# cvlab-stonybrook/s-volsdf

Measured on AMD Instinct MI355X. Metric: rendered rays/sec (1024-ray batch, 128 samples), higher is better.
Workload: dtype f32 (every product, forward and backward, as three fp16 MFMA products of two-piece fp16 operands with f32 accumulate; activation blocks hold both pieces: float32 accuracy class); 1 GPU; configs[1]: VolOpt.train_step (forward + MVS prior lookup + loss + backward + clip/guard/Adam), train mode, fast=1: 1024 rays/GPU x 128 coarse + 98 composited samples + 2048 eikonal points, 8x256 SDF MLP + 4x256 radiance MLP; mode=train, mlp_precision=fp16x2, launch=eager launches, rays_per_gpu=1024, rays_total=1024

## Files before the change

### include/svolsdf_hip.h

```cpp
#ifndef SVOLSDF_HIP_H
#define SVOLSDF_HIP_H

#include <stddef.h>
#include <stdint.h>

#ifdef __cplusplus
extern "C" {
#endif

int svs_version(void);
const char* svs_last_error_string(void);

int svs_set_deterministic(int on);
int svs_get_deterministic(void);

int svs_rays_from_uv(const float* uv, const float* pose, const float* intrinsics, int n_rays, float* ray_dirs,
                     float* cam_loc, float* depth_scale, void* hip_stream);

int svs_eikonal_points(const float* uniform_points, const float* cam_loc, const float* z_eik, const float* ray_dirs,
                       int n_rays, float* points, void* hip_stream);
int svs_stage_in(const void* pinned_host, void* device, size_t bytes, void* hip_stream);
int svs_split_last(const float* z, int n_rays, int n, float* head, float* last, void* hip_stream);

enum { SVS_MMA_F32 = 0, SVS_MMA_F16X2 = 1, SVS_MMA_F16X2_HALF = 2 };
// ... 53 lines not shown
                   float* zbuf, float* feat_bar, float* absmax, void* hip_stream);
int svs_bg_sdf_bwd(int n_points, const float* d_out0, const float* feat_bar, const float* hbuf, const float* ghat7,
                   const float* stream, int precision, float* abuf, float* sbar_out, float* absmax, void* hip_stream);
int svs_composite_bg(int n_rays, int n_samples, int n_bg, const float* z, const float* z_max, const float* sdf,
                     const float* rgb, const float* normals, const float* depth_scale, const float* beta_param,
                     float beta_min, const float* z_bg, const float* bg_out0, const float* bg_rgb, const float* bg_depth,
                     float* weights, float* bg_trans, float* bg_weights, float* rgb_values, float* depth_values,
                     float* depth_values_all, float* depth_vals, float* normal_map, void* hip_stream);
int svs_composite_bg_bwd(int n_rays, int n_samples, int n_bg, const float* z, const float* z_max, const float* sdf,
                         const float* rgb, const float* depth_scale, const float* beta_param, float beta_min,
                         const float* z_bg, const float* bg_out0, const float* bg_rgb, const float* d_rgb_values,
                         const float* d_weights, const float* d_depth_values, const float* d_depth_all,
                         const float* bg_depth, float* d_sdf, float* d_rgb,
                         float* d_bg_out0, float* d_bg_rgb, float* d_beta_ray, float* d_beta_param, void* hip_stream);

typedef struct svs_wgrad_job {
  const float *a0, *b0; long long sa0, sb0;
  const float *a1, *b1; long long sa1, sb1;
  const float* b_extra; long long s_extra;
  int n_points, ldw;
  float *dW, *db;
  const float* absmax;
  const float *rec0, *rec1;
} svs_wgrad_job;
int svs_wgrad_multi(const svs_wgrad_job* jobs, int n_jobs, int precision, void* hip_stream);
int svs_wgrad(const float* a0, const float* b0, long long sa0, long long sb0, const float* a1, const float* b1,
              long long sa1, long long sb1, const float* b_extra, long long s_extra, int n_points, int precision,
              const float* absmax, const float* rec0, const float* rec1, float* dW, int ldw, float* db, void* hip_stream);

size_t svs_block_bytes(int n_points, int blocks_per_tile);
size_t svs_rgb_zbuf_bytes(int n_points);
size_t svs_sdf_ubuf_bytes(int n_points);
size_t svs_sdf_gbuf_bytes(int n_points);
int svs_rgb_bwd(int n_points, const float* d_rgb, const float* rgb, const float* rbuf, const float* stream, int precision,
                float* zbuf, float* feat_bar, float* d_normals, float* absmax, void* hip_stream);
int svs_sdf_bwd_a(const float* points, int n_points, const float* cam, int cam_stride, const float* dirs, const float* z,
                  int S, int n_rays, const float* d_grad, const unsigned char* clamp_mask, const float* hbuf,
                  const float* gbuf, const float* stream, int precision, float* ubuf, float* a2buf, float* pebuf,
                  float* absmax, void* hip_stream);
int svs_sdf_bwd_b(int n_points, const float* d_sdf, const unsigned char* clamp_mask, const float* feat_bar,
                  int n_feat_points, const float* hbuf, const float* gbuf, const float* a2buf, const float* ubuf,
                  const float* stream, int precision, float* abuf, float* sbar_out, float* absmax, void* hip_stream);
int svs_lin8_row0_grad(const float* hbuf, const float* ubuf, const float* sbar, int n_points, int precision, float* out257,
                       void* hip_stream);
int svs_unpack_wgrad(const float* dWk, const float* dbk, int ldw, int map, int rows, int cols, int row_off,
                     const float* weight_v, const float* weight_g, const float* row0, float* grad_v, float* grad_g,
                     float* grad_b, void* hip_stream);
// ... 205 lines not shown
```

### s-volsdf_amd/csrc/svs_wgrad.hip

```cpp
#include "svs_common.h"
#include "svs_mlp_layout.h"
#include "svs_ticket.h"
#include <cstdlib>

namespace svs {
namespace wgrad {

struct Pair {
  const float* a;
  const float* b;
  size_t stride_a, stride_b;
};

struct Args {
  Pair p[2];
  int n_pairs;
  int n_tiles;
  int n_valid_points;
  const float* b_extra;
  size_t stride_extra;
  float* dW;
  int ldw;
  float* db;
  det::Ticket ticket;
// ... 137 lines not shown
  __builtin_amdgcn_sched_barrier(0);
}
__device__ __forceinline__ unsigned lds_addr(const void* p) {
  return (unsigned)(unsigned long long)SVS_LDS(const void, p);
}

__device__ __forceinline__ void scale_from_absmax(const float* absmax, float& s, float& inv_s) {
  s = 1.0f; inv_s = 1.0f;
  if (!absmax) return;
  int e = (int)((__float_as_uint(*absmax) >> 23) & 0xff);
  e = e < 16 ? 16 : (e > 250 ? 250 : e);
  s = __uint_as_float((unsigned)(268 - e) << 23);
  inv_s = __uint_as_float((unsigned)(e - 14) << 23);
}

struct Job {
  Pair p[2];
  const float* rec[2];
  int n_pairs;
  int n_tiles;
  int n_valid_points;
  int b_tiles;
  int col0;
  float* dW;
  int ldw;
  float* db;
  const float* absmax;
  int wg_begin, wg_count;
  det::Ticket ticket;
};
constexpr int kMaxJobs = 20;
struct MultiArgs { Job job[kMaxJobs]; int n_jobs; int touch; int reverse; };
static_assert(sizeof(MultiArgs) <= 4096, "kernel arguments");

constexpr int kThreadsW = 512;

typedef const __attribute__((address_space(1))) void* gvoid;

template <bool GP>
__global__ __launch_bounds__(kThreadsW, 1) void wgrad_h2_multi_kernel(MultiArgs ma) {
  typedef Ring<GP> R;
  constexpr int kSlot = R::kSlot, kSlotAll = R::kSlotAll, kRing = R::kRing, kAhead = R::kAhead, kB = R::kB;
  extern __shared__ __attribute__((aligned(16))) unsigned char smem_h2[];
  int jj = 0;
  for (int q = 1; q < ma.n_jobs; ++q) if ((int)blockIdx.x >= ma.job[q].wg_begin) jj = q;
  const Job& a = ma.job[jj];
  const int wg = (int)blockIdx.x - a.wg_begin, nwg = a.wg_count;
  const int tid = threadIdx.x, lane = tid & 63;
  const int wave = __builtin_amdgcn_readfirstlane(tid >> 6);
  const bool narrow = a.b_tiles == 1;
  float s_grad, inv_s;
  scale_from_absmax(a.absmax, s_grad, inv_s);

  f32x16 acc[8];
#pragma unroll
  for (int i = 0; i < 8; ++i) acc[i] = (f32x16)(0.0f);
  float bsum = 0.0f;

  unsigned char* ring = smem_h2;

  const int rq = (lane & 15) >> 2, rp = lane & 3, rg = (lane >> 4) & 1, rh = lane >> 5;
  const int rd0 = 1024 * rg + 256 * rh + 128 * rg + 64 * (rp & 1) + 16 * rq + 8 * (rp >> 1);
  const int a_rd = 2048 * wave + rd0;
  const int rx0 = 64 * (8 * rh + rq) + 32 * rg + 8 * rp, rx1 = rx0 + 64 * 4;
  const int wp = lane & 31, whf = lane >> 5;
  const int wxoff = 64 * wp + 16 * (wave & 3) + 8 * whf;

  const bool two_pairs = a.n_pairs == 2;
  const int my_tiles = a.n_tiles > wg ? (a.n_tiles - 1 - wg) / nwg + 1 : 0;
  const int n_items = two_pairs ? 2 * my_tiles : my_tiles;
  const int n_valid = a.n_valid_points;
  const bool has_db = a.db != nullptr;
  const bool rev = ma.reverse != 0;
  const float* const pa0 = a.p[0].a; const float* const pb0 = a.p[0].b;
  const float* const pa1 = a.p[1].a; const float* const pb1 = a.p[1].b;
  const size_t sa0 = a.p[0].stride_a, sb0 = a.p[0].stride_b, sa1 = a.p[1].stride_a, sb1 = a.p[1].stride_b;
  const float* const rec0 = a.rec[0]; const float* const rec1 = a.rec[1];
  const bool has_scale = a.absmax != nullptr;
  auto tile_of = [&](int item) {
    const int k = two_pairs ? item >> 1 : item;
    return rev ? wg + (my_tiles - 1 - k) * nwg : wg + k * nwg;
  };

  auto issue = [&](int item) {
    const int t = tile_of(item), pi = two_pairs ? item & 1 : 0;
    const float* pa = (pi ? pa1 : pa0) + (size_t)t * (pi ? sa1 : sa0);
    const float* pb = (pi ? pb1 : pb0) + (size_t)t * (pi ? sb1 : sb0);
    unsigned char* slot = ring + (item % kRing) * kSlotAll;
#pragma unroll
    for (int j = 0; j < 2 * R::kPlanes; ++j) {
      const int piece = wave + 8 * j;
      __builtin_amdgcn_global_load_lds((gvoid)(reinterpret_cast<const f32x4*>(pa) + piece * 64 + lane),
                                       SVS_LDS(void, slot + piece * 1024), 16, 0, 0);
      if (!narrow)
        __builtin_amdgcn_global_load_lds((gvoid)(reinterpret_cast<const f32x4*>(pb) + piece * 64 + lane),
                                         SVS_LDS(void, slot + kB + piece * 1024), 16, 0, 0);
    }
    if (narrow)
      __builtin_amdgcn_global_load_lds((gvoid)(reinterpret_cast<const f32x4*>(pb) + (wave & 3) * 64 + lane),
                                       SVS_LDS(void, slot + kB + (wave & 3) * 1024), 16, 0, 0);
    if (has_scale)
      __builtin_amdgcn_global_load_lds((gvoid)((pi ? rec1 : rec0) + (size_t)t * 64 + lane),
                                       SVS_LDS(void, slot + kSlot + wave * 256), 4, 0, 0);
  };
  unsigned sink = 0;
  auto touch = [&](int item) {
    const int t = tile_of(item), pi = two_pairs ? item & 1 : 0;
    const Pair& p = a.p[pi];
    constexpr int kLines = R::kPlanes * (kPlane / 128);
    const int nb = narrow ? 32 : kLines;
    const float* q = tid < kLines ? p.a + (size_t)t * p.stride_a + tid * 32
                                  : p.b + (size_t)t * p.stride_b + (tid - kLines) * 32;
    if (tid < kLines + nb) asm volatile("global_load_dword %0, %1, off" : "+v"(sink) : "v"(q) : "memory");
  };
  const int ops = (narrow ? 2 * R::kPlanes + 1 : 4 * R::kPlanes) + (has_scale ? 1 : 0);

  auto stage_factors = [&](int item) {
    unsigned char* slot = ring + (item % kRing) * kSlotAll;
    const int t = tile_of(item);
    const int live = n_valid - t * 32;
    float f = 1.0f;
    if (has_scale) {
      float rec;
      lds_read32(rec, lds_addr(slot + kSlot + wave * 256 + 4 * wp));
      lds_wait();
      const unsigned eb = (__float_as_uint(rec) >> 23) & 0xff;
      if (eb >= 20 && eb <= 240) f = __builtin_fminf(s_grad * __uint_as_float((254u << 23) - __float_as_uint(rec)), 32768.0f);
    }
    if (wp >= live) f = 0.0f;
    if (lane < 32) asm volatile("ds_write_b16 %0, %1" :: "v"(lds_addr(slot + kSlot + kRecBytes + wave * 64 + 2 * lane)), "v"((_Float16)f) : "memory");
  };
  auto stage_narrow = [&](int item) {
    unsigned char* slot = ring + (item % kRing) * kSlotAll;
    if (tid < 256) {
      f32x4 v;
      lds_read128(v, lds_addr(slot + kB + tid * 16));
      lds_wait();
      f16x4 hi, mid;
#pragma unroll
      for (int j = 0; j < 4; ++j) {
        const _Float16 h = (_Float16)v[j];
        hi[j] = h;
        mid[j] = (_Float16)(v[j] - (float)h);
      }
      *SVS_LDS(f16x4, slot + kB + kNarrowImg + wxoff) = hi;
      *SVS_LDS(f16x4, slot + kB + kNarrowImg + kExtraPiece + wxoff) = mid;
    }
  };

  const f16x2 one2 = {(_Float16)1.0f, (_Float16)1.0f};

  for (int i0 = 0; i0 < kAhead && i0 < n_items; ++i0) issue(i0);
  const bool touching = GP && ma.touch;
  bool touched = false;
  if (touching && kAhead < n_items) { touch(kAhead); touched = true; }
  auto pre_stage = [&](int it) {
    const int left = n_items - 1 - it;
    const int later = (left < kAhead - 1 ? left : kAhead - 1) * ops;
    if (later == 10) asm volatile("s_waitcnt vmcnt(10)" ::: "memory");
    else if (later == 8) asm volatile("s_waitcnt vmcnt(8)" ::: "memory");
    else if (later == 6) asm volatile("s_waitcnt vmcnt(6)" ::: "memory");
    else if (later == 5) asm volatile("s_waitcnt vmcnt(5)" ::: "memory");
    else if (later == 4) asm volatile("s_waitcnt vmcnt(4)" ::: "memory");
    else if (later == 3) asm volatile("s_waitcnt vmcnt(3)" ::: "memory");
    else if (touched) asm volatile("s_waitcnt vmcnt(1)" ::: "memory");
    else asm volatile("s_waitcnt vmcnt(0)" ::: "memory");
    stage_factors(it);
  };
  for (int item = 0; item < n_items; ++item) {
    const int pi = two_pairs ? item & 1 : 0;
    const bool p0 = pi == 0;
    pre_stage(item);
    asm volatile("s_waitcnt lgkmcnt(0)\n\ts_barrier" ::: "memory");
    if (narrow) {
      stage_narrow(item);
      asm volatile("s_waitcnt lgkmcnt(0)\n\ts_barrier" ::: "memory");
    }
    auto issue_next = [&]() {
      if (item + kAhead < n_items) issue(item + kAhead);
      touched = false;
      if (touching && item + kAhead + 1 < n_items) { touch(item + kAhead + 1); touched = true; }
    };
    const unsigned la = lds_addr(ring + (item % kRing) * kSlotAll);
    const unsigned lb = la + kB;
    const unsigned ftab = la + kSlot + kRecBytes + wave * 64;
    const unsigned nimg = lb + kNarrowImg;
    const bool want_bias = has_db && p0;
    const bool two = narrow;
    Frag fa2[2], fam2[2];
    f32x4 fraw2[2];
#pragma unroll
    for (int ks = 0; ks < 2; ++ks) {
      tr_issue(fa2[ks], la + 512 * ks + a_rd, la + 512 * ks + (a_rd ^ 128));
      if (GP) tr_issue(fam2[ks], la + kPlane + 512 * ks + a_rd, la + kPlane + 512 * ks + (a_rd ^ 128));
      lds_read128(fraw2[ks], ftab + 32 * ks + 16 * rh);
    }
    issue_next();
    lds_wait();
#pragma unroll
    for (int ks = 0; ks < 2; ++ks) {
      const f16x8 ah = frag_of(fa2[ks]) * __builtin_bit_cast(f16x8, fraw2[ks]);
      const f16x8 am = GP ? frag_of(fam2[ks]) * __builtin_bit_cast(f16x8, fraw2[ks]) : ah;
      if (want_bias) {
#pragma unroll
        for (int j = 0; j < 4; ++j) {
          const f16x2 h2v = {ah[2 * j], ah[2 * j + 1]};
          bsum = __builtin_amdgcn_fdot2(h2v, one2, bsum, false);
          if (GP) {
            const f16x2 m2v = {am[2 * j], am[2 * j + 1]};
            bsum = __builtin_amdgcn_fdot2(m2v, one2, bsum, false);
          }
        }
      }
#pragma unroll
      for (int i = 0; i < 8; ++i) {
        if (i > 0 && narrow) break;
        Frag fh, fm;
        if (!narrow) {
          const unsigned rd = lb + 2048 * i + 512 * ks + rd0;
          tr_issue(fh, rd, rd ^ 128);
          if (GP) tr_issue(fm, rd + kPlane, (rd ^ 128) + kPlane);
        } else {
          tr_issue(fh, nimg + ks * 1024 + rx0, nimg + ks * 1024 + rx1);
          tr_issue(fm, nimg + kExtraPiece + ks * 1024 + rx0, nimg + kExtraPiece + ks * 1024 + rx1);
        }
        lds_wait();
        if (two || GP) acc[i] = __builtin_amdgcn_mfma_f32_32x32x16_f16(ah, frag_of(fm), acc[i], 0, 0, 0);
        if (GP) acc[i] = __builtin_amdgcn_mfma_f32_32x32x16_f16(am, frag_of(fh), acc[i], 0, 0, 0);
        acc[i] = __builtin_amdgcn_mfma_f32_32x32x16_f16(ah, frag_of(fh), acc[i], 0, 0, 0);
      }
    }
  }
  asm volatile("s_waitcnt vmcnt(0)" :: "v"(sink) : "memory");
  const int half = lane >> 5, col = lane & 31;
  det::wait_turn(a.ticket, wg);
#pragma unroll
  for (int i = 0; i < 8; ++i) {
    if (i > 0 && narrow) break;
#pragma unroll
    for (int r = 0; r < 16; ++r) {
      const int row = 32 * wave + rho(r) + 4 * half;
      const int c = a.col0 + 32 * i + col;
      if (c < a.ldw) atomicAdd(&a.dW[(size_t)row * a.ldw + c], acc[i][r] * inv_s);
    }
  }
  if (a.db) {
    bsum += __shfl_xor(bsum, 32);
    if (half == 0) atomicAdd(&a.db[32 * wave + col], bsum * inv_s);
  }
  det::pass_turn(a.ticket, wg);
}

}

}
}

using namespace svs;
using namespace svs::wgrad;
namespace h2 = svs::wgrad::h2;

extern "C" {

struct svs_wgrad_job {
  const float *a0, *b0; long long sa0, sb0;
  const float *a1, *b1; long long sa1, sb1;
  const float* b_extra; long long s_extra;
  int n_points, ldw;
  float *dW, *db;
  const float* absmax;
  const float *rec0, *rec1;
};

int svs_wgrad_multi(const svs_wgrad_job* jobs, int n_jobs, int precision, void* hip_stream) {
  if (!jobs || n_jobs < 1) { set_error("svs_wgrad_multi: no jobs"); return SVS_EINVAL; }
  int n_expanded = 0;
  for (int j = 0; j < n_jobs; ++j) n_expanded += jobs[j].b_extra ? 2 : 1;
  if (n_expanded > h2::kMaxJobs) { set_error("svs_wgrad_multi: at most %d jobs (b_extra counts twice)", h2::kMaxJobs); return SVS_EINVAL; }
  for (int j = 0; j < n_jobs; ++j) {
    const svs_wgrad_job& q = jobs[j];
    if (!q.a0 || !q.b0 || !q.dW || q.n_points <= 0 || q.ldw < 256 || q.ldw > 288 || (q.b_extra && q.ldw < 288) || (q.a1 && !q.b1)) {
      set_error("svs_wgrad_multi: bad argument in job %d", j); return SVS_EINVAL;
    }
    if (mlp::is_h2(precision) && q.absmax && (!q.rec0 || (q.a1 && !q.rec1))) {
      set_error("svs_wgrad_multi: job %d has absmax but no scale records", j); return SVS_EINVAL;
    }
  }
  hipStream_t s = (hipStream_t)hip_stream;
  if (mlp::is_h2(precision)) {
    const bool gp = precision == mlp::kFmtF16x2;
    h2::MultiArgs ma;
    int n = 0;
    long long work[h2::kMaxJobs], total = 0;
    for (int j = 0; j < n_jobs; ++j) {
      const svs_wgrad_job& q = jobs[j];
      h2::Job& J = ma.job[n];
      J.p[0] = Pair{q.a0, q.b0, (size_t)q.sa0, (size_t)q.sb0};
      J.rec[0] = q.rec0; J.rec[1] = q.rec1;
      J.n_pairs = 1;
      if (q.a1) { J.p[1] = Pair{q.a1, q.b1, (size_t)q.sa1, (size_t)q.sb1}; J.n_pairs = 2; }
      else { J.p[1] = J.p[0]; J.rec[1] = J.rec[0]; }
      J.n_tiles = (q.n_points + 31) / 32; J.n_valid_points = q.n_points;
      J.b_tiles = 8; J.col0 = 0; J.dW = q.dW; J.ldw = q.ldw; J.db = q.db; J.absmax = q.absmax;
      work[n] = (long long)J.n_tiles * J.n_pairs * 10;
      total += work[n++];
      if (q.b_extra) {
        h2::Job& X = ma.job[n];
        X = J;
        X.p[0].b = q.b_extra; X.p[0].stride_b = (size_t)q.s_extra; X.n_pairs = 1;
        X.b_tiles = 1; X.col0 = 256; X.db = nullptr;
        work[n] = (long long)X.n_tiles * 6;
        total += work[n++];
      }
    }
    ma.n_jobs = n;
    static const int touch_env = [] { const char* e = getenv("SVS_WGRAD_TOUCH"); return e ? atoi(e) : 0; }();
    ma.touch = touch_env;
    static const int reverse_env = [] { const char* e = getenv("SVS_WGRAD_REVERSE"); return e ? atoi(e) : 0; }();
    ma.reverse = reverse_env;
    (void)total;
    const int n_wg_total = 256;
    int count[h2::kMaxJobs];
    int used = 0;
    for (int j = 0; j < n; ++j) { count[j] = 1; ++used; }
    while (used < n_wg_total) {
      int best = -1;
      double load = 0.0;
      for (int j = 0; j < n; ++j) {
        if (count[j] >= ma.job[j].n_tiles) continue;
        const double l = (double)work[j] / count[j];
        if (l > load) { load = l; best = j; }
      }
      if (best < 0) break;
      ++count[best]; ++used;
// ... 72 lines not shown
```

### s-volsdf_amd/svs_hip/lib.py

```python
import ctypes
import os
from ctypes import POINTER, c_char_p, c_double, c_float, c_int, c_longlong, c_size_t, c_void_p

_HERE = os.path.dirname(os.path.abspath(__file__))
LIB_PATH = os.environ.get("SVS_LIB_PATH") or os.path.join(os.path.dirname(_HERE), "lib", "libsvolsdf_hip.so")

_lib = None


class SvsError(RuntimeError):
    pass


_P = c_void_p
_PP = POINTER(c_void_p)

class WGradJob(ctypes.Structure):
    _fields_ = [("a0", ctypes.c_void_p), ("b0", ctypes.c_void_p), ("sa0", ctypes.c_longlong), ("sb0", ctypes.c_longlong),
                ("a1", ctypes.c_void_p), ("b1", ctypes.c_void_p), ("sa1", ctypes.c_longlong), ("sb1", ctypes.c_longlong),
                ("b_extra", ctypes.c_void_p), ("s_extra", ctypes.c_longlong),
                ("n_points", ctypes.c_int), ("ldw", ctypes.c_int),
                ("dW", ctypes.c_void_p), ("db", ctypes.c_void_p), ("absmax", ctypes.c_void_p),
                ("rec0", ctypes.c_void_p), ("rec1", ctypes.c_void_p)]


class UnpackJob(ctypes.Structure):
    _fields_ = [("dWk", ctypes.c_void_p), ("dbk", ctypes.c_void_p), ("ldw", ctypes.c_int), ("map", ctypes.c_int),
                ("rows", ctypes.c_int), ("cols", ctypes.c_int), ("row_off", ctypes.c_int),
                ("weight_v", ctypes.c_void_p), ("weight_g", ctypes.c_void_p), ("row0", ctypes.c_void_p),
                ("grad_v", ctypes.c_void_p), ("grad_g", ctypes.c_void_p), ("grad_b", ctypes.c_void_p)]


SIGNATURES = {
    "svs_version": (c_int, []),
    "svs_set_deterministic": (c_int, [c_int]),
    "svs_get_deterministic": (c_int, []),
    "svs_last_error_string": (c_char_p, []),
    "svs_rays_from_uv": (c_int, [_P, _P, _P, c_int, _P, _P, _P, _P]),
    "svs_stream_bytes": (c_size_t, [c_int]),
    "svs_pack_stream": (c_int, [c_int, c_int, _PP, _PP, _PP, _P, _P, _P]),
    "svs_pack_workspace_bytes": (c_size_t, []),
    "svs_sdf_vals": (c_int, [_P, c_int, _P, c_int, _P, _P, c_int, c_int, _P, c_int, c_float, c_float, c_int, _P, _P,
                             c_int, c_int, _P]),
    "svs_sdf_hbuf_bytes": (c_size_t, [c_int]),
    "svs_sdf_gbuf_bytes": (c_size_t, [c_int]),
    "svs_feat_tiles_bytes": (c_size_t, [c_int]),
# ... 5 lines not shown
    "svs_block_bytes": (c_size_t, [c_int, c_int]),
    "svs_rgb_zbuf_bytes": (c_size_t, [c_int]),
    "svs_sdf_ubuf_bytes": (c_size_t, [c_int]),
    "svs_rgb_bwd": (c_int, [c_int, _P, _P, _P, _P, c_int, _P, _P, _P, _P, _P]),
    "svs_sdf_bwd_a": (c_int, [_P, c_int, _P, c_int, _P, _P, c_int, c_int, _P, _P, _P, _P, _P, c_int, _P, _P, _P,
                              _P, _P]),
    "svs_sdf_bwd_b": (c_int, [c_int, _P, _P, _P, c_int, _P, _P, _P, _P, _P, c_int, _P, _P, _P, _P]),
    "svs_lin8_row0_grad": (c_int, [_P, _P, _P, c_int, c_int, _P, _P]),
    "svs_unpack_wgrad": (c_int, [_P, _P, c_int, c_int, c_int, c_int, c_int, _P, _P, _P, _P, _P, _P, _P]),
    "svs_unpack_wgrad_multi": (c_int, [_P, c_int, _P]),
    "svs_sampler_ctl_bytes": (c_size_t, [c_int, c_int]),
    "svs_sampler_ctl_stride": (c_int, []),
    "svs_sampler_cap": (c_int, []),
    "svs_sampler_max_new": (c_int, []),
    "svs_sampler_init": (c_int, [_P, c_int, _P, c_int, c_int, c_float, c_float, c_int, c_float, _P, c_float, c_int,
                                 _P, _P, _P, _P, c_int, _P, _P]),
    "svs_sampler_round": (c_int, [c_int, c_int, c_int, c_int, c_int, c_int, c_int, _P, c_float, c_float, c_int, c_float,
                                  c_float, _P, _P, _P, _P, _P, _P, _P, c_int, _P, _P, _P, _P, _P, _P, _P, _P, _P, _P]),
    "svs_composite": (c_int, [c_int, c_int, _P, _P, _P, _P, _P, _P, c_float, _P, _P, _P, _P, _P, _P]),
    "svs_composite_bwd": (c_int, [c_int, c_int, _P, _P, _P, _P, _P, c_float, _P, _P, _P, _P, _P, _P, _P, _P]),
    "svs_wgrad": (c_int, [_P, _P, ctypes.c_longlong, ctypes.c_longlong, _P, _P, ctypes.c_longlong, ctypes.c_longlong,
                          _P, ctypes.c_longlong, c_int, c_int, _P, _P, _P, _P, c_int, _P, _P]),
    "svs_wgrad_multi": (c_int, [_P, c_int, c_int, _P]),
    "svs_bg_points": (c_int, [_P, c_int, _P, c_int, c_int, _P, c_float, _P, _P, _P, _P]),
    "svs_bg_sdf_eval": (c_int, [_P, c_int, _P, c_int, _P, _P, _P, _P, _P, _P]),
    "svs_bg_rgb_bwd": (c_int, [c_int, _P, _P, _P, _P, c_int, _P, _P, _P, _P]),
    "svs_bg_sdf_bwd": (c_int, [c_int, _P, _P, _P, _P, _P, c_int, _P, _P, _P, _P]),
    "svs_bg_rbuf_bytes": (c_size_t, [c_int]),
    "svs_bg_rgb_eval": (c_int, [c_int, _P, c_int, _P, _P, c_int, _P, _P, _P]),
    "svs_composite_bg_bwd": (c_int, [c_int, c_int, c_int, _P, _P, _P, _P, _P, _P, c_float, _P, _P, _P, _P, _P, _P, _P, _P,
                                     _P, _P, _P, _P, _P, _P, _P]),
    "svs_composite_bg": (c_int, [c_int, c_int, c_int, _P, _P, _P, _P, _P, _P, _P, c_float, _P, _P, _P, _P,
                                 _P, _P, _P, _P, _P, _P, _P, _P, _P]),
    "svs_adam_workspace_bytes": (c_size_t, []),
    "svs_clip_guard_adam": (c_int, [_P, _P, _P, _P, ctypes.c_longlong, c_int, _P, c_double, c_double, c_double, c_double,
                                    c_double, _P, _P, _P]),
    "svs_cost_lookup": (c_int, [_P, _P, _P, _P, c_int, c_int, c_int, c_int, c_int, c_float, c_float, POINTER(c_float),
                                _PP, _PP, _PP, POINTER(c_int), _P, _P, _P, _P, _P]),
    "svs_loss": (c_int, [c_int, c_int, c_int, _P, _P, _P, _P, _P, _P, _P, c_float, c_float, c_float, c_float, c_float,
                         c_float, c_int, c_float, c_int, c_int, _P, _P, _P, _P, _P, _P, _P, _P]),
    "svs_loss_workspace_bytes": (c_size_t, [c_int, c_int]),
    "svs_conv2d": (c_int, [_P, _P, _P, _P, c_int, _P, c_int, c_int, c_int, c_int, c_int, c_int, c_int, _P]),
    "svs_featurenet_fpn_workspace_bytes": (c_size_t, [c_int, c_int, c_int]),
    "svs_featurenet_fpn": (c_int, [_P, c_int, c_int, c_int, _P, _P, _P, _P, _P, _P, _P]),
    "svs_featurenet_fpn2": (c_int, [_P, c_int, c_int, c_int, _P, _P, _P, _P, _P, _P, _P, _P]),
    "svs_conv2d_mfma_supported": (c_int, [c_int, c_int, c_int, c_int]),
# ... 102 lines not shown
    "svs_lpips_workspace_bytes": (c_size_t, [c_int, c_int, c_int]),
    "svs_lpips_score": (c_int, [_P, _P, _P, c_int, c_int, c_int, _P, _P, _P, _P]),
})

ABI_VERSION = 101


def load():
    global _lib
    if _lib is not None:
        return _lib
    import torch
    if not os.path.exists(LIB_PATH):
        raise SvsError(f"{LIB_PATH} not found: run `python s-volsdf_amd/build.py` (there is no CPU fallback)")
    lib = ctypes.CDLL(LIB_PATH)
    for name, (res, args) in SIGNATURES.items():
        fn = getattr(lib, name)
        fn.restype = res
        fn.argtypes = args
    have = lib.svs_version()
    if have != ABI_VERSION:
        raise SvsError(f"{LIB_PATH} has ABI version {have}, this binding was written against {ABI_VERSION}: "
                       "rebuild with `python s-volsdf_amd/build.py --force`")
    if os.environ.get("SVS_DETERMINISTIC") == "1":
        lib.svs_set_deterministic(1)
    _lib = lib
    return lib


def deterministic():
    return bool(load().svs_get_deterministic())


def check(rc, what=""):
    if rc != 0:
        msg = load().svs_last_error_string()
        raise SvsError(f"{what} failed (code {rc}): {msg.decode() if msg else ''}")
```

### s-volsdf_amd/svs_hip/train.py

```python
import ctypes
import os

import torch

from . import lib as _lib
from .ops import _f32, _ptr, _ptr_array, _stream, default_precision, is_h2, F16X2, F16X2_HALF

KBLOCK = 128 * 64
KREC = 64


def block_stride(n_points):
    return ((n_points + 127) // 128) * 4 * KBLOCK
LDW = 288


def n_tiles_padded(n_points):
    return ((n_points + 127) // 128) * 4


def record_off(n_points, n_blocks, block):
    T = n_tiles_padded(n_points)
    return n_blocks * T * KBLOCK + block * T * KREC


def _off(t, n_floats):
    return t.data_ptr() + 4 * n_floats


class TrainStreams:
    def __init__(self, device, precision=None):
        L = _lib.load()
        self.precision = default_precision() if precision is None else int(precision)
        self.sdf = torch.empty(L.svs_stream_bytes(2) // 4, device=device)
        self.rgb = torch.empty(L.svs_stream_bytes(4) // 4, device=device)
        self.ws = torch.empty(L.svs_pack_workspace_bytes() // 4, device=device)

    def pack(self, sdf_params, rgb_params):
        L = _lib.load()
        sv, sg, sb = [[_f32(t) for t in x] if x is not None else None for x in sdf_params]
        rv, rg, rb = [[_f32(t) for t in x] if x is not None else None for x in rgb_params]
        self._keep = (sv, sg, sb, rv, rg, rb)
        st = _stream()
        _lib.check(L.svs_pack_stream(2, self.precision, _ptr_array(sv), _ptr_array(sg) if sg else None, _ptr_array(sb), _ptr(self.ws),
                                     _ptr(self.sdf), st), "svs_pack_stream(sdf train)")
        _lib.check(L.svs_pack_stream(4, self.precision, _ptr_array(rv), _ptr_array(rg) if rg else None, _ptr_array(rb), _ptr(self.ws),
                                     _ptr(self.rgb), st), "svs_pack_stream(rgb bwd)")


class WGradAccum:
    def __init__(self, device):
        n = [14 * 256 * LDW, 14 * 256, 260, 4]
        self.flat = torch.zeros(sum(n), device=device)
        parts = torch.split(self.flat, n)
        self.dWk = parts[0].view(14, 256, LDW)
        self.dbk = parts[1].view(14, 256)
        self.row0 = parts[2][:257]
        self.absmax = parts[3]

    def zero(self):
        self.flat.zero_()


def _unpack_all(jobs):
    L = _lib.load()
    val = lambda x: x.value if isinstance(x, ctypes.c_void_p) else x
    arr = (_lib.UnpackJob * len(jobs))(*[_lib.UnpackJob(*[val(x) for x in j]) for j in jobs])
    _lib.check(L.svs_unpack_wgrad_multi(ctypes.cast(arr, ctypes.c_void_p), len(jobs), _stream()), "svs_unpack_wgrad_multi")


# ... 69 lines not shown

    def grad_extra_out(self, n_total, n_main):
        self._alloc(n_total, n_main)
        return self.d_grad_full[n_main:]

    def accumulate(self, keep, d_rgb, d_sdf, d_grad_extra, wait=True, side=True, defer_wgrad=False, extra=None):
        L = _lib.load()
        src = keep["src"]
        n_total, n_main = src.n, keep["rgb"].shape[0]
        if n_main % 32:
            raise NotImplementedError("rays*samples of a group must be a multiple of 32")
        self._alloc(n_total, n_main)
        dev, acc, S = self.dev, self.accum, self.streams
        LS = block_stride(n_total)
        hbuf, gbuf, mask = keep["hbuf"], keep["gbuf"], keep["clamp_mask"]
        rbuf, feat = keep["rbuf"], keep["feat_tiles"]

        prec = S.precision
        h2 = is_h2(prec)

        def addr(x):
            return x.value if isinstance(x, ctypes.c_void_p) else x

        def job(slot, n_pts, amax, a0, sa0, b0, sb0, a1=None, sa1=0, b1=None, sb1=0, extra=None, sx=0, rec0=None, rec1=None):
            return _lib.WGradJob(addr(a0), addr(b0), sa0, sb0, addr(a1), addr(b1), sa1, sb1,
                                 addr(extra), sx, n_pts, LDW, addr(_off(acc.dWk, slot * 256 * LDW)),
                                 addr(_off(acc.dbk, slot * 256)), addr(_off(acc.absmax, amax)) if h2 else None,
                                 addr(rec0) if h2 else None, addr(rec1) if h2 else None)

        def wgrad_multi(cached):
            arr, n = cached
            _lib.check(L.svs_wgrad_multi(arr, n, prec, _stream()), "svs_wgrad_multi")

        def job_list(key, build):
            hit = self._job_cache.get(key)
            if hit is None:
                if len(self._job_cache) >= 64:
                    self._job_cache.clear()
                hit = self._job_cache[key] = build()
            return hit

        def job_array(key, own, more):
            key = ("arr",) + key + ((more["key"],) if more else ())
            hit = self._job_cache.get(key)
            if hit is None:
                return self._cache_jobs(key, list(own) + (list(more["jobs"]) if more else []))
            return hit[:2]

        d_rgb = _f32(d_rgb)
        d_grad = self.d_grad_full
        d_normals = d_grad[:n_main]
# ... 6 lines not shown
                                 _ptr(self.feat_bar), _ptr(d_normals), _ptr(acc.absmax) if h2 else None, _stream()),
                   "svs_rgb_bwd")
        if d_sdf is not None and d_sdf.data_ptr() == self.d_sdf_full.data_ptr() and d_sdf.numel() == n_main:
            d_sdf_full = self.d_sdf_full
        else:
            d_sdf_full = torch.zeros(n_total, device=dev)
            if d_sdf is not None:
                d_sdf_full[:n_main] = _f32(d_sdf).reshape(-1)
        main = torch.cuda.current_stream()
        if self._side is None:
            self._side = torch.cuda.Stream(device=dev)
        if os.environ.get("SVS_RGB_WGRAD_SIDE", "1") == "0":
            side = False
        side_stream = self._side if side else main
        rkey = ("rgb", n_main, prec, self.zbuf.data_ptr(), feat.data_ptr(), rbuf.data_ptr(), acc.dWk.data_ptr())

        def rgb_jobs():
            LSm = block_stride(n_main)
            zrec = lambda l: _off(self.zbuf, record_off(n_main, 5, l))
            jobs = [job(9, n_main, 1, _off(self.zbuf, 0), KBLOCK, _ptr(feat), KBLOCK, extra=_off(rbuf, 4 * LSm), sx=1024,
                        rec0=zrec(0))]
            for l in range(1, 5):
                jobs.append(job(9 + l, n_main, 1, _off(self.zbuf, l * LSm), KBLOCK, _off(rbuf, (l - 1) * LSm), KBLOCK,
                                rec0=zrec(l)))
            return jobs

        deferred = None
        if defer_wgrad:
            ev_rgb = torch.cuda.Event(); ev_rgb.record(main)
            deferred = dict(rgb=dict(jobs=job_list(rkey, rgb_jobs), key=rkey), ev_rgb=ev_rgb)
            join = None
        else:
            fork = torch.cuda.Event(); fork.record(main)
            with torch.cuda.stream(side_stream):
                if side:
                    side_stream.wait_event(fork)
                if extra is not None:
                    side_stream.wait_event(extra["ev_rgb"])
                wgrad_multi(job_array(rkey, job_list(rkey, rgb_jobs), extra["rgb"] if extra else None))
                join = torch.cuda.Event(); join.record(side_stream)
        st = _stream()
        _lib.check(L.svs_sdf_bwd_a(*src.args(), _ptr(d_grad), _ptr(mask), _ptr(hbuf), _ptr(gbuf), _ptr(S.sdf), prec,
                                   _ptr(self.ubuf), _ptr(self.a2buf), _ptr(self.pebuf),
                                   _ptr(acc.absmax) if h2 else None, st), "svs_sdf_bwd_a")
        _lib.check(L.svs_sdf_bwd_b(n_total, _ptr(d_sdf_full), _ptr(mask), _ptr(self.feat_bar), n_main, _ptr(hbuf),
                                   _ptr(gbuf), _ptr(self.a2buf), _ptr(self.ubuf), _ptr(S.sdf), prec, _ptr(self.abuf),
                                   _ptr(self.sbar), _ptr(acc.absmax) if h2 else None, st),
                   "svs_sdf_bwd_b")
        _lib.check(L.svs_lin8_row0_grad(_ptr(hbuf), _ptr(self.ubuf), _ptr(self.sbar), n_total, prec, _ptr(acc.row0),
                                        _stream()), "svs_lin8_row0_grad")
        ev = self.timer_events = ([torch.cuda.Event(enable_timing=True) for _ in range(2)] if self.time_wgrad else None)
        if ev:
            ev[0].record()
        skey = ("sdf", n_total, n_main, prec, self.abuf.data_ptr(), self.ubuf.data_ptr(), self.pebuf.data_ptr(),
                hbuf.data_ptr(), gbuf.data_ptr(), self.feat_bar.data_ptr(), acc.dWk.data_ptr())

        def sdf_jobs():
            arec = lambda l: _off(self.abuf, record_off(n_total, 8, l))
            urec = lambda l: _off(self.ubuf, record_off(n_total, 9, l))
            second = lambda l: dict(a1=_off(gbuf, l * LS), sa1=KBLOCK, b1=_off(self.ubuf, l * LS), sb1=KBLOCK, rec1=urec(l))
            jobs = [job(0, n_total, 0, _off(self.abuf, 0), KBLOCK, _ptr(self.pebuf), KBLOCK, rec0=arec(0), **second(0))]
            for l in range(1, 8):
                jobs.append(job(l, n_total, 0, _off(self.abuf, l * LS), KBLOCK, _off(hbuf, (l - 1) * LS), KBLOCK, rec0=arec(l),
                                **second(l)))
            jobs.append(job(8, n_main, 2, _ptr(self.feat_bar), KBLOCK, _off(hbuf, 7 * LS), KBLOCK,
                            rec0=_off(self.feat_bar, record_off(n_main, 1, 0))))
            return jobs

        if defer_wgrad:
            deferred["sdf"] = dict(jobs=job_list(skey, sdf_jobs), key=skey)
            deferred["ev_all"] = torch.cuda.Event(); deferred["ev_all"].record(main)
            deferred["hold"] = self._hold = (d_grad, d_sdf_full, d_normals, d_rgb)
            return deferred
        if extra is not None:
            main.wait_event(extra["ev_all"])
        wgrad_multi(job_array(skey, job_list(skey, sdf_jobs), extra["sdf"] if extra else None))
        if ev:
            ev[1].record()
        if wait and side:
            main.wait_event(join)
        self._hold = (d_grad, d_sdf_full, d_normals, d_rgb)
        return join

    def run(self, sdf_params, rgb_params, keep, d_rgb, d_sdf, d_grad_extra, out=None):
# ... 5 lines not shown

class BgBackward:
    BGRBUF = KBLOCK + 1024

    def __init__(self, device, precision=None):
        L = _lib.load()
        self.dev = device
        self.precision = default_precision() if precision is None else int(precision)
        self.sdf_stream = torch.empty(L.svs_stream_bytes(6) // 4, device=device)
        self.rgb_stream = torch.empty(L.svs_stream_bytes(8) // 4, device=device)
        self.ws = torch.empty(L.svs_pack_workspace_bytes() // 4, device=device)
        n = [11 * 256 * LDW, 11 * 256, 260, 4]
        self.flat = torch.zeros(sum(n), device=device)
        parts = torch.split(self.flat, n)
        self.dWk = parts[0].view(11, 256, LDW)
        self.dbk = parts[1].view(11, 256)
        self.row0 = parts[2][:257]
        self.absmax = parts[3]
        self._scratch = {}

    def pack(self, sdf_wb, rgb_wb):
        L = _lib.load()
        self._keep = []
        for which, (w, b), stream in ((6, sdf_wb, self.sdf_stream), (8, rgb_wb, self.rgb_stream)):
            w, b = [_f32(t) for t in w], [_f32(t) for t in b]
            self._keep += [w, b]
            _lib.check(L.svs_pack_stream(which, self.precision, _ptr_array(w), None, _ptr_array(b), _ptr(self.ws), _ptr(stream),
                                         _stream()), "svs_pack_stream(bg backward)")

    def zero(self):
        self.flat.zero_()

    def _alloc(self, n, slot):
        cur = self._scratch.get(slot)
        if cur is not None and cur[0] == n:
            return cur[1:]
        L = _lib.load()
        z = lambda nbytes: torch.zeros(nbytes // 4, device=self.dev)
        cur = (n, z(L.svs_block_bytes(n, 2)),
               z(L.svs_block_bytes(n, 1)), z(L.svs_block_bytes(n, 8)), z(L.svs_block_bytes(n, 1) // (128 * 2)))
        self._scratch[slot] = cur
        return cur[1:]

    def accumulate(self, keep, d_bg_rgb, d_bg_out0, slot=0):
        L = _lib.load()
        P = keep["bg_rgb"].shape[0]
        zbuf, feat_bar, abuf, sbar = self._alloc(P, slot)
        st = _stream()
        hbuf, ghat7, pebuf, rbuf, feat = keep["bg_hbuf"], keep["bg_ghat7"], keep["bg_pebuf"], keep["bg_rbuf"], keep["bg_feat"]
        d_bg_rgb, d_bg_out0 = _f32(d_bg_rgb), _f32(d_bg_out0)
        prec = self.precision
        _lib.check(L.svs_bg_rgb_bwd(P, _ptr(d_bg_rgb), _ptr(keep["bg_rgb"]), _ptr(rbuf), _ptr(self.rgb_stream), prec, _ptr(zbuf),
                                    _ptr(feat_bar), _ptr(self.absmax), st), "svs_bg_rgb_bwd")
        _lib.check(L.svs_bg_sdf_bwd(P, _ptr(d_bg_out0), _ptr(feat_bar), _ptr(hbuf), _ptr(ghat7), _ptr(self.sdf_stream), prec,
                                    _ptr(abuf), _ptr(sbar), _ptr(self.absmax), st), "svs_bg_sdf_bwd")
        _lib.check(L.svs_lin8_row0_grad(_ptr(hbuf), None, _ptr(sbar), P, prec, _ptr(self.row0), st), "svs_lin8_row0_grad")
        LS, Z2 = block_stride(P), 2 * KBLOCK
        T = n_tiles_padded(P)

        def addr(x):
            return x.value if isinstance(x, ctypes.c_void_p) else x

        def job(slot, amax, a0, sa0, b0, sb0, rec0, extra=None, sx=0):
            return _lib.WGradJob(addr(a0), addr(b0), sa0, sb0, None, None, 0, 0, addr(extra), sx, P, LDW,
                                 addr(_off(self.dWk, slot * 256 * LDW)), addr(_off(self.dbk, slot * 256)),
                                 addr(_off(self.absmax, amax)), addr(rec0), None)

        arec = lambda l: _off(abuf, record_off(P, 8, l))
        jobs = [job(0, 0, _off(abuf, 0), KBLOCK, _ptr(pebuf), KBLOCK, arec(0))]
        for l in range(1, 8):
            jobs.append(job(l, 0, _off(abuf, l * LS), KBLOCK, _off(hbuf, (l - 1) * LS), KBLOCK, arec(l)))
        jobs.append(job(8, 2, _ptr(feat_bar), KBLOCK, _off(hbuf, 7 * LS), KBLOCK, _off(feat_bar, record_off(P, 1, 0))))
        zrec = lambda b: _off(zbuf, 2 * T * KBLOCK + b * T * KREC)
        jobs.append(job(9, 1, _off(zbuf, 0), Z2, _ptr(feat), KBLOCK, zrec(0), extra=_off(rbuf, KBLOCK), sx=self.BGRBUF))
        jobs.append(job(10, 1, _off(zbuf, KBLOCK), Z2, _ptr(rbuf), self.BGRBUF, zrec(1)))
        arr = (_lib.WGradJob * len(jobs))(*jobs)
        _lib.check(L.svs_wgrad_multi(ctypes.cast(arr, ctypes.c_void_p), len(jobs), prec, st), "svs_wgrad_multi(bg)")
        self._hold = getattr(self, "_hold", {})
        self._hold[slot] = (d_bg_rgb, d_bg_out0)

    def finalize(self, sdf_wb, rgb_wb, out=None):
        res, jobs, keep = [], [], []
        for gi, ((w, b), base) in enumerate(((sdf_wb, 0), (rgb_wb, 9))):
            group = []
            for l in range(len(w)):
                rows, cols = w[l].shape
                gw, gb = out[gi][l] if out is not None else (torch.empty(rows, cols, device=self.dev), torch.empty(rows, device=self.dev))
                is_sdf = gi == 0
                mp = 3 if (is_sdf and l == 4) else (4 if (not is_sdf and l == 0) else 0)
                row_off = 1 if (is_sdf and l == 8) else 0
                row0 = _ptr(self.row0) if (is_sdf and l == 8) else None
                wl = _f32(w[l])
                keep.append(wl)
                jobs.append((_off(self.dWk, (base + l) * 256 * LDW), _off(self.dbk, (base + l) * 256), LDW, mp, rows, cols, row_off,
                             _ptr(wl), None, row0, _ptr(gw), None, _ptr(gb)))
                group.append((gw, gb))
            res.append(group)
        _unpack_all(jobs)
# ... 19 lines not shown
```

Baseline: 301,700 rays/s.

## Skip padded rows and columns in thin weight-gradient jobs and price work by shape

Weight-gradient jobs now carry real output rows and input columns. The multi-job kernel uses these to skip loading padding pieces, idle waves beyond the real rows, and limit B tiles to the real column count. Affected layers are the first SDF layer (39 inputs) and the last radiance layer (3 outputs). Per-job work estimates become shape-dependent prices, so workgroups are split across jobs by actual cost. This adds wait-count logic that varies with load counts and an ABI struct-size check, which could mis-synchronise if the vmcnt accounting is wrong.

```diff
diff --git a/include/svolsdf_hip.h b/include/svolsdf_hip.h
--- a/include/svolsdf_hip.h
+++ b/include/svolsdf_hip.h
@@ -99,7 +99,9 @@
   float *dW, *db;
   const float* absmax;
   const float *rec0, *rec1;
+  int a_rows, b_cols;
 } svs_wgrad_job;
+int svs_wgrad_job_bytes(void);
 int svs_wgrad_multi(const svs_wgrad_job* jobs, int n_jobs, int precision, void* hip_stream);
 int svs_wgrad(const float* a0, const float* b0, long long sa0, long long sb0, const float* a1, const float* b1,
               long long sa1, long long sb1, const float* b_extra, long long s_extra, int n_points, int precision,
diff --git a/s-volsdf_amd/csrc/svs_wgrad.hip b/s-volsdf_amd/csrc/svs_wgrad.hip
--- a/s-volsdf_amd/csrc/svs_wgrad.hip
+++ b/s-volsdf_amd/csrc/svs_wgrad.hip
@@ -183,6 +183,8 @@
   int n_valid_points;
   int b_tiles;
   int col0;
+  int a_rows;
+  int b_cols;
   float* dW;
   int ldw;
   float* db;
@@ -194,9 +196,35 @@
 struct MultiArgs { Job job[kMaxJobs]; int n_jobs; int touch; int reverse; };
 static_assert(sizeof(MultiArgs) <= 4096, "kernel arguments");
 
+constexpr int kPriceWide = 100, kPriceNarrow = 60;
+#ifndef SVS_WGRAD_PRICE_FIXED
+#define SVS_WGRAD_PRICE_FIXED 55
+#endif
+constexpr int kPriceFixed = SVS_WGRAD_PRICE_FIXED;
+inline int item_price(int a_rows, int b_cols) {
+  const int waves_per_simd = ((a_rows + 31) / 32 + 3) / 4, b_tiles = (b_cols + 31) / 32;
+  return kPriceFixed + (kPriceWide - kPriceFixed) * waves_per_simd * b_tiles / 16;
+}
 constexpr int kThreadsW = 512;
 
 typedef const __attribute__((address_space(1))) void* gvoid;
+
+#define SVS_WGRAD_B_TILE(i, nar)                                                                                      \
+  {                                                                                                                   \
+    Frag fh, fm;                                                                                                      \
+    if (!(nar)) {                                                                                                     \
+      const unsigned rd = lb + 2048 * (i) + 512 * ks + rd0;                                                           \
+      tr_issue(fh, rd, rd ^ 128);                                                                                     \
+      if (GP) tr_issue(fm, rd + kPlane, (rd ^ 128) + kPlane);                                                         \
+    } else {                                                                                                          \
+      tr_issue(fh, nimg + ks * 1024 + rx0, nimg + ks * 1024 + rx1);                                                   \
+      tr_issue(fm, nimg + kExtraPiece + ks * 1024 + rx0, nimg + kExtraPiece + ks * 1024 + rx1);                       \
+    }                                                                                                                 \
+    lds_wait();                                                                                                       \
+    if ((nar) || GP) acc[i] = __builtin_amdgcn_mfma_f32_32x32x16_f16(ah, frag_of(fm), acc[i], 0, 0, 0);               \
+    if (GP) acc[i] = __builtin_amdgcn_mfma_f32_32x32x16_f16(am, frag_of(fh), acc[i], 0, 0, 0);                        \
+    acc[i] = __builtin_amdgcn_mfma_f32_32x32x16_f16(ah, frag_of(fh), acc[i], 0, 0, 0);                                \
+  }
 
 template <bool GP>
 __global__ __launch_bounds__(kThreadsW, 1) void wgrad_h2_multi_kernel(MultiArgs ma) {
@@ -210,6 +238,9 @@
   const int tid = threadIdx.x, lane = tid & 63;
   const int wave = __builtin_amdgcn_readfirstlane(tid >> 6);
   const bool narrow = a.b_tiles == 1;
+  const int a_rows = a.a_rows, npa = (a_rows + 15) >> 4;
+  const int nbt = narrow ? 1 : (a.b_cols + 31) >> 5, npb = narrow ? 0 : 2 * nbt;
+  const bool active = 32 * wave < a_rows;
   float s_grad, inv_s;
   scale_from_absmax(a.absmax, s_grad, inv_s);
 
@@ -222,7 +253,7 @@
 
   const int rq = (lane & 15) >> 2, rp = lane & 3, rg = (lane >> 4) & 1, rh = lane >> 5;
   const int rd0 = 1024 * rg + 256 * rh + 128 * rg + 64 * (rp & 1) + 16 * rq + 8 * (rp >> 1);
-  const int a_rd = 2048 * wave + rd0;
+  const int a_rd = 2048 * wave + ((2 * wave + 1 < npa) ? rd0 : rd0 - (1024 + 128) * rg);
   const int rx0 = 64 * (8 * rh + rq) + 32 * rg + 8 * rp, rx1 = rx0 + 64 * 4;
   const int wp = lane & 31, whf = lane >> 5;
   const int wxoff = 64 * wp + 16 * (wave & 3) + 8 * whf;
@@ -250,10 +281,11 @@
     unsigned char* slot = ring + (item % kRing) * kSlotAll;
 #pragma unroll
     for (int j = 0; j < 2 * R::kPlanes; ++j) {
-      const int piece = wave + 8 * j;
-      __builtin_amdgcn_global_load_lds((gvoid)(reinterpret_cast<const f32x4*>(pa) + piece * 64 + lane),
-                                       SVS_LDS(void, slot + piece * 1024), 16, 0, 0);
-      if (!narrow)
+      const int piece = wave + 8 * j, pin = piece & 15;
+      if (pin < npa)
+        __builtin_amdgcn_global_load_lds((gvoid)(reinterpret_cast<const f32x4*>(pa) + piece * 64 + lane),
+                                         SVS_LDS(void, slot + piece * 1024), 16, 0, 0);
+      if (pin < npb)
         __builtin_amdgcn_global_load_lds((gvoid)(reinterpret_cast<const f32x4*>(pb) + piece * 64 + lane),
                                          SVS_LDS(void, slot + kB + piece * 1024), 16, 0, 0);
     }
@@ -274,7 +306,7 @@
                                   : p.b + (size_t)t * p.stride_b + (tid - kLines) * 32;
     if (tid < kLines + nb) asm volatile("global_load_dword %0, %1, off" : "+v"(sink) : "v"(q) : "memory");
   };
-  const int ops = (narrow ? 2 * R::kPlanes + 1 : 4 * R::kPlanes) + (has_scale ? 1 : 0);
+  const int ops = R::kPlanes * ((wave < npa) + (wave + 8 < npa) + (wave < npb) + (wave + 8 < npb)) + (narrow ? 1 : 0) + (has_scale ? 1 : 0);
 
   auto stage_factors = [&](int item) {
     unsigned char* slot = ring + (item % kRing) * kSlotAll;
@@ -318,12 +350,14 @@
   auto pre_stage = [&](int it) {
     const int left = n_items - 1 - it;
     const int later = (left < kAhead - 1 ? left : kAhead - 1) * ops;
-    if (later == 10) asm volatile("s_waitcnt vmcnt(10)" ::: "memory");
-    else if (later == 8) asm volatile("s_waitcnt vmcnt(8)" ::: "memory");
-    else if (later == 6) asm volatile("s_waitcnt vmcnt(6)" ::: "memory");
+    if (later >= 10) asm volatile("s_waitcnt vmcnt(10)" ::: "memory");
+    else if (later >= 8) asm volatile("s_waitcnt vmcnt(8)" ::: "memory");
+    else if (later >= 6) asm volatile("s_waitcnt vmcnt(6)" ::: "memory");
     else if (later == 5) asm volatile("s_waitcnt vmcnt(5)" ::: "memory");
     else if (later == 4) asm volatile("s_waitcnt vmcnt(4)" ::: "memory");
     else if (later == 3) asm volatile("s_waitcnt vmcnt(3)" ::: "memory");
+    else if (later == 2) asm volatile("s_waitcnt vmcnt(2)" ::: "memory");
+    else if (later == 1) asm volatile("s_waitcnt vmcnt(1)" ::: "memory");
     else if (touched) asm volatile("s_waitcnt vmcnt(1)" ::: "memory");
     else asm volatile("s_waitcnt vmcnt(0)" ::: "memory");
     stage_factors(it);
@@ -346,8 +380,8 @@
     const unsigned lb = la + kB;
     const unsigned ftab = la + kSlot + kRecBytes + wave * 64;
     const unsigned nimg = lb + kNarrowImg;
+    if (!active) { issue_next(); continue; }
     const bool want_bias = has_db && p0;
-    const bool two = narrow;
     Frag fa2[2], fam2[2];
     f32x4 fraw2[2];
 #pragma unroll
@@ -375,42 +409,35 @@
       }
 #pragma unroll
       for (int i = 0; i < 8; ++i) {
-        if (i > 0 && narrow) break;
-        Frag fh, fm;
-        if (!narrow) {
-          const unsigned rd = lb + 2048 * i + 512 * ks + rd0;
-          tr_issue(fh, rd, rd ^ 128);
-          if (GP) tr_issue(fm, rd + kPlane, (rd ^ 128) + kPlane);
-        } else {
-          tr_issue(fh, nimg + ks * 1024 + rx0, nimg + ks * 1024 + rx1);
-          tr_issue(fm, nimg + kExtraPiece + ks * 1024 + rx0, nimg + kExtraPiece + ks * 1024 + rx1);
-        }
-        lds_wait();
-        if (two || GP) acc[i] = __builtin_amdgcn_mfma_f32_32x32x16_f16(ah, frag_of(fm), acc[i], 0, 0, 0);
-        if (GP) acc[i] = __builtin_amdgcn_mfma_f32_32x32x16_f16(am, frag_of(fh), acc[i], 0, 0, 0);
-        acc[i] = __builtin_amdgcn_mfma_f32_32x32x16_f16(ah, frag_of(fh), acc[i], 0, 0, 0);
+        if (i >= nbt) break;
+        SVS_WGRAD_B_TILE(i, i == 0 && narrow)
       }
     }
   }
   asm volatile("s_waitcnt vmcnt(0)" :: "v"(sink) : "memory");
   const int half = lane >> 5, col = lane & 31;
+  const int c_end = narrow ? a.ldw : (a.col0 + a.b_cols < a.ldw ? a.col0 + a.b_cols : a.ldw);
   det::wait_turn(a.ticket, wg);
-#pragma unroll
-  for (int i = 0; i < 8; ++i) {
-    if (i > 0 && narrow) break;
-#pragma unroll
-    for (int r = 0; r < 16; ++r) {
-      const int row = 32 * wave + rho(r) + 4 * half;
-      const int c = a.col0 + 32 * i + col;
-      if (c < a.ldw) atomicAdd(&a.dW[(size_t)row * a.ldw + c], acc[i][r] * inv_s);
-    }
-  }
-  if (a.db) {
-    bsum += __shfl_xor(bsum, 32);
-    if (half == 0) atomicAdd(&a.db[32 * wave + col], bsum * inv_s);
+  if (active) {
+#pragma unroll
+    for (int i = 0; i < 8; ++i) {
+      if (i >= nbt) break;
+#pragma unroll
+      for (int r = 0; r < 16; ++r) {
+        const int row = 32 * wave + rho(r) + 4 * half;
+        const int c = a.col0 + 32 * i + col;
+        if (c < c_end && row < a_rows) atomicAdd(&a.dW[(size_t)row * a.ldw + c], acc[i][r] * inv_s);
+      }
+    }
+    if (a.db) {
+      bsum += __shfl_xor(bsum, 32);
+      if (half == 0 && 32 * wave + col < a_rows) atomicAdd(&a.db[32 * wave + col], bsum * inv_s);
+    }
   }
   det::pass_turn(a.ticket, wg);
 }
+
+#undef SVS_WGRAD_B_TILE
 
 }
 
@@ -431,7 +458,10 @@
   float *dW, *db;
   const float* absmax;
   const float *rec0, *rec1;
+  int a_rows, b_cols;
 };
+
+int svs_wgrad_job_bytes(void) { return (int)sizeof(svs_wgrad_job); }
 
 int svs_wgrad_multi(const svs_wgrad_job* jobs, int n_jobs, int precision, void* hip_stream) {
   if (!jobs || n_jobs < 1) { set_error("svs_wgrad_multi: no jobs"); return SVS_EINVAL; }
@@ -442,6 +472,10 @@
     const svs_wgrad_job& q = jobs[j];
     if (!q.a0 || !q.b0 || !q.dW || q.n_points <= 0 || q.ldw < 256 || q.ldw > 288 || (q.b_extra && q.ldw < 288) || (q.a1 && !q.b1)) {
       set_error("svs_wgrad_multi: bad argument in job %d", j); return SVS_EINVAL;
+    }
+    if (q.a_rows < 0 || q.a_rows > 256 || q.b_cols < 0 || q.b_cols > 256) {
+      set_error("svs_wgrad_multi: job %d: a_rows = %d, b_cols = %d, both must be 0 (= 256) or 1..256", j, q.a_rows, q.b_cols);
+      return SVS_EINVAL;
     }
     if (mlp::is_h2(precision) && q.absmax && (!q.rec0 || (q.a1 && !q.rec1))) {
       set_error("svs_wgrad_multi: job %d has absmax but no scale records", j); return SVS_EINVAL;
@@ -463,14 +497,15 @@
       else { J.p[1] = J.p[0]; J.rec[1] = J.rec[0]; }
       J.n_tiles = (q.n_points + 31) / 32; J.n_valid_points = q.n_points;
       J.b_tiles = 8; J.col0 = 0; J.dW = q.dW; J.ldw = q.ldw; J.db = q.db; J.absmax = q.absmax;
-      work[n] = (long long)J.n_tiles * J.n_pairs * 10;
+      J.a_rows = q.a_rows ? q.a_rows : 256; J.b_cols = q.b_cols ? q.b_cols : 256;
+      work[n] = (long long)J.n_tiles * J.n_pairs * h2::item_price(J.a_rows, J.b_cols);
       total += work[n++];
       if (q.b_extra) {
         h2::Job& X = ma.job[n];
         X = J;
         X.p[0].b = q.b_extra; X.p[0].stride_b = (size_t)q.s_extra; X.n_pairs = 1;
-        X.b_tiles = 1; X.col0 = 256; X.db = nullptr;
-        work[n] = (long long)X.n_tiles * 6;
+        X.b_tiles = 1; X.col0 = 256; X.db = nullptr; X.b_cols = 256;
+        work[n] = (long long)X.n_tiles * h2::kPriceNarrow;
         total += work[n++];
       }
     }
diff --git a/s-volsdf_amd/svs_hip/lib.py b/s-volsdf_amd/svs_hip/lib.py
--- a/s-volsdf_amd/svs_hip/lib.py
+++ b/s-volsdf_amd/svs_hip/lib.py
@@ -21,7 +21,8 @@
                 ("b_extra", ctypes.c_void_p), ("s_extra", ctypes.c_longlong),
                 ("n_points", ctypes.c_int), ("ldw", ctypes.c_int),
                 ("dW", ctypes.c_void_p), ("db", ctypes.c_void_p), ("absmax", ctypes.c_void_p),
-                ("rec0", ctypes.c_void_p), ("rec1", ctypes.c_void_p)]
+                ("rec0", ctypes.c_void_p), ("rec1", ctypes.c_void_p),
+                ("a_rows", ctypes.c_int), ("b_cols", ctypes.c_int)]
 
 
 class UnpackJob(ctypes.Structure):
@@ -73,6 +74,7 @@
     "svs_wgrad": (c_int, [_P, _P, ctypes.c_longlong, ctypes.c_longlong, _P, _P, ctypes.c_longlong, ctypes.c_longlong,
                           _P, ctypes.c_longlong, c_int, c_int, _P, _P, _P, _P, c_int, _P, _P]),
     "svs_wgrad_multi": (c_int, [_P, c_int, c_int, _P]),
+    "svs_wgrad_job_bytes": (c_int, []),
     "svs_bg_points": (c_int, [_P, c_int, _P, c_int, c_int, _P, c_float, _P, _P, _P, _P]),
     "svs_bg_sdf_eval": (c_int, [_P, c_int, _P, c_int, _P, _P, _P, _P, _P, _P]),
     "svs_bg_rgb_bwd": (c_int, [c_int, _P, _P, _P, _P, c_int, _P, _P, _P, _P]),
@@ -221,6 +223,9 @@
     if have != ABI_VERSION:
         raise SvsError(f"{LIB_PATH} has ABI version {have}, this binding was written against {ABI_VERSION}: "
                        "rebuild with `python s-volsdf_amd/build.py --force`")
+    if lib.svs_wgrad_job_bytes() != ctypes.sizeof(WGradJob):
+        raise SvsError(f"{LIB_PATH}: svs_wgrad_job has {lib.svs_wgrad_job_bytes()} bytes, this binding's has "
+                       f"{ctypes.sizeof(WGradJob)}: rebuild with `python s-volsdf_amd/build.py --force`")
     if os.environ.get("SVS_DETERMINISTIC") == "1":
         lib.svs_set_deterministic(1)
     _lib = lib
diff --git a/s-volsdf_amd/svs_hip/train.py b/s-volsdf_amd/svs_hip/train.py
--- a/s-volsdf_amd/svs_hip/train.py
+++ b/s-volsdf_amd/svs_hip/train.py
@@ -46,6 +46,10 @@
                                      _ptr(self.sdf), st), "svs_pack_stream(sdf train)")
         _lib.check(L.svs_pack_stream(4, self.precision, _ptr_array(rv), _ptr_array(rg) if rg else None, _ptr_array(rb), _ptr(self.ws),
                                      _ptr(self.rgb), st), "svs_pack_stream(rgb bwd)")
+
+
+SDF_IN = 3 + 3 * 2 * 6
+RGB_OUT = 3
 
 
 class WGradAccum:
@@ -161,11 +165,12 @@
         def addr(x):
             return x.value if isinstance(x, ctypes.c_void_p) else x
 
-        def job(slot, n_pts, amax, a0, sa0, b0, sb0, a1=None, sa1=0, b1=None, sb1=0, extra=None, sx=0, rec0=None, rec1=None):
+        def job(slot, n_pts, amax, a0, sa0, b0, sb0, a1=None, sa1=0, b1=None, sb1=0, extra=None, sx=0, rec0=None, rec1=None,
+                a_rows=0, b_cols=0):
             return _lib.WGradJob(addr(a0), addr(b0), sa0, sb0, addr(a1), addr(b1), sa1, sb1,
                                  addr(extra), sx, n_pts, LDW, addr(_off(acc.dWk, slot * 256 * LDW)),
                                  addr(_off(acc.dbk, slot * 256)), addr(_off(acc.absmax, amax)) if h2 else None,
-                                 addr(rec0) if h2 else None, addr(rec1) if h2 else None)
+                                 addr(rec0) if h2 else None, addr(rec1) if h2 else None, a_rows, b_cols)
 
         def wgrad_multi(cached):
             arr, n = cached
@@ -218,7 +223,7 @@
                         rec0=zrec(0))]
             for l in range(1, 5):
                 jobs.append(job(9 + l, n_main, 1, _off(self.zbuf, l * LSm), KBLOCK, _off(rbuf, (l - 1) * LSm), KBLOCK,
-                                rec0=zrec(l)))
+                                rec0=zrec(l), a_rows=RGB_OUT if l == 4 else 0))
             return jobs
 
         deferred = None
@@ -255,7 +260,8 @@
             arec = lambda l: _off(self.abuf, record_off(n_total, 8, l))
             urec = lambda l: _off(self.ubuf, record_off(n_total, 9, l))
             second = lambda l: dict(a1=_off(gbuf, l * LS), sa1=KBLOCK, b1=_off(self.ubuf, l * LS), sb1=KBLOCK, rec1=urec(l))
-            jobs = [job(0, n_total, 0, _off(self.abuf, 0), KBLOCK, _ptr(self.pebuf), KBLOCK, rec0=arec(0), **second(0))]
+            jobs = [job(0, n_total, 0, _off(self.abuf, 0), KBLOCK, _ptr(self.pebuf), KBLOCK, rec0=arec(0), b_cols=SDF_IN,
+                        **second(0))]
             for l in range(1, 8):
                 jobs.append(job(l, n_total, 0, _off(self.abuf, l * LS), KBLOCK, _off(hbuf, (l - 1) * LS), KBLOCK, rec0=arec(l),
                                 **second(l)))
@@ -307,6 +313,7 @@
     def pack(self, sdf_wb, rgb_wb):
         L = _lib.load()
         self._keep = []
+        self._thin = (int(sdf_wb[0][0].shape[1]), int(rgb_wb[0][-1].shape[0]))
         for which, (w, b), stream in ((6, sdf_wb, self.sdf_stream), (8, rgb_wb, self.rgb_stream)):
             w, b = [_f32(t) for t in w], [_f32(t) for t in b]
             self._keep += [w, b]
@@ -346,19 +353,20 @@
         def addr(x):
             return x.value if isinstance(x, ctypes.c_void_p) else x
 
-        def job(slot, amax, a0, sa0, b0, sb0, rec0, extra=None, sx=0):
+        def job(slot, amax, a0, sa0, b0, sb0, rec0, extra=None, sx=0, a_rows=0, b_cols=0):
             return _lib.WGradJob(addr(a0), addr(b0), sa0, sb0, None, None, 0, 0, addr(extra), sx, P, LDW,
                                  addr(_off(self.dWk, slot * 256 * LDW)), addr(_off(self.dbk, slot * 256)),
-                                 addr(_off(self.absmax, amax)), addr(rec0), None)
-
+                                 addr(_off(self.absmax, amax)), addr(rec0), None, a_rows, b_cols)
+
+        pe_rows, rgb_rows = getattr(self, "_thin", (0, 0))
         arec = lambda l: _off(abuf, record_off(P, 8, l))
-        jobs = [job(0, 0, _off(abuf, 0), KBLOCK, _ptr(pebuf), KBLOCK, arec(0))]
+        jobs = [job(0, 0, _off(abuf, 0), KBLOCK, _ptr(pebuf), KBLOCK, arec(0), b_cols=pe_rows)]
         for l in range(1, 8):
             jobs.append(job(l, 0, _off(abuf, l * LS), KBLOCK, _off(hbuf, (l - 1) * LS), KBLOCK, arec(l)))
         jobs.append(job(8, 2, _ptr(feat_bar), KBLOCK, _off(hbuf, 7 * LS), KBLOCK, _off(feat_bar, record_off(P, 1, 0))))
         zrec = lambda b: _off(zbuf, 2 * T * KBLOCK + b * T * KREC)
         jobs.append(job(9, 1, _off(zbuf, 0), Z2, _ptr(feat), KBLOCK, zrec(0), extra=_off(rbuf, KBLOCK), sx=self.BGRBUF))
-        jobs.append(job(10, 1, _off(zbuf, KBLOCK), Z2, _ptr(rbuf), self.BGRBUF, zrec(1)))
+        jobs.append(job(10, 1, _off(zbuf, KBLOCK), Z2, _ptr(rbuf), self.BGRBUF, zrec(1), a_rows=rgb_rows))
         arr = (_lib.WGradJob * len(jobs))(*jobs)
         _lib.check(L.svs_wgrad_multi(ctypes.cast(arr, ctypes.c_void_p), len(jobs), prec, st), "svs_wgrad_multi(bg)")
         self._hold = getattr(self, "_hold", {})
```

Result: no change. 301,000 rays/s (-0.2%).
